# yancie-yjr/StreamYOLO

Measured on AMD Instinct MI355X. Metric: frame-pairs/sec (600x960) StreamYOLO-l fwd+bwd, higher is better.
Workload: dtype bf16; 1 GPU; StreamYOLO-l 600x960 training step: dual-frame forward + TAL loss + backward, 8 frame pairs/GPU/step, random-init synthetic weights (utils/synth.py); per_gpu_batch=8, global_batch=8, parallelism=dp1, hipgraph=False, launch_tape=True, optimizer_in_step=False, u8_input=False

## Files before the change

### streamyolo_amd/csrc/api_misc.hip

```cpp
#include "sy_device.h"
#include "../../include/streamyolo_hip.h"

extern "C" const char* sy_version(void) {
#ifdef SY_EMU
    return "streamyolo-hip 0.1 (SIMT-EMULATOR TEST BUILD - not a product binary)";
#else
    return "streamyolo-hip 0.1 (gfx950)";
#endif
}
extern "C" int sy_abi_version(void) { return SY_ABI_VERSION; }

namespace {

template <typename T> __device__ __forceinline__ void put(void* base, long long i, float v) {
    reinterpret_cast<typename T::elem*>(base)[i] = T::from_f32(v);
}
template <typename T> __device__ __forceinline__ long long frag_index(int row, int tap, int c, int taps, int kc) {
    constexpr int EPC = T::kEPC, BK = 4 * EPC;
    const int cslab = c / BK, within = c % BK;
    const int g = within / (2 * EPC), half = (within / EPC) & 1, e = within % EPC;
    const int ct = row >> 5, r = row & 31, nslab = kc / BK;
    return ((((((long long)ct * nslab + cslab) * taps + tap) * 2 + g) * 2 + half) * 32 + r) * EPC + e;
}

constexpr int kPackTile = 32, kPackTaps = 9;

template <typename T> __device__ void pack_tile(const sy_pack_entry& e, int tile, float (*lds)[kPackTile][kPackTile + 1]) {
    const int tiles_ci = (e.ci_n + kPackTile - 1) / kPackTile;
    const int co0 = (tile / tiles_ci) * kPackTile, ci0 = (tile % tiles_ci) * kPackTile;
    const int taps = e.taps;
    const int a_l = threadIdx.x >> 5, b_l = threadIdx.x & 31;
    for (int pass = 0; pass < kPackTile / 8; ++pass) {
        const int col = a_l + 8 * pass, co = co0 + col, ci = ci0 + b_l;
        const bool ok = co < e.co_n && ci < e.ci_n;
        const float* src = e.w + ((long long)co * e.ci_n + ci) * taps;
        const int row = e.r0 + co;
        for (int t = 0; t < taps; ++t) {
            const float v = ok ? src[t] : 0.0f;
            lds[t][col][b_l] = v;
            if (!ok) continue;
            if (e.packed != nullptr) put<T>(e.packed, ((long long)row * taps + t) * e.CI + ci, v);
            if (e.frag != nullptr) put<T>(e.frag, frag_index<T>(row, t, ci, taps, e.CI), v);
        }
    }
    __syncthreads();
    if (e.packed_t == nullptr && e.frag_t == nullptr) return;
    for (int pass = 0; pass < kPackTile / 8; ++pass) {
        const int cil = a_l + 8 * pass, ci = ci0 + cil, co = co0 + b_l;
        if (co >= e.co_n || ci >= e.ci_n) continue;
        const int row = e.r0 + co;
        for (int t = 0; t < taps; ++t) {
            const float v = lds[t][b_l][cil];
            if (e.packed_t != nullptr) put<T>(e.packed_t, ((long long)ci * taps + t) * e.R_t + row, v);
            if (e.frag_t != nullptr) put<T>(e.frag_t, frag_index<T>(ci, t, row, taps, e.R_t), v);
        }
    }
}

__global__ __launch_bounds__(256) void pack_weights_kernel(const sy_pack_entry* entries, int n_entries) {
    SY_TL_BEGIN(15);
    __shared__ float lds[kPackTaps][kPackTile][kPackTile + 1];
    int lo = 0, hi = n_entries - 1;
    while (lo < hi) {
        const int mid = (lo + hi + 1) >> 1;
        if (entries[mid].tile0 <= (int)blockIdx.x) lo = mid; else hi = mid - 1;
    }
    const sy_pack_entry e = entries[lo];
    const int tile = (int)blockIdx.x - e.tile0;
    const int tiles = ((e.co_n + kPackTile - 1) / kPackTile) * ((e.ci_n + kPackTile - 1) / kPackTile);
    if (tile >= tiles || e.taps > kPackTaps) return;
    switch (e.dtype) {
        case SY_DT_BF16: pack_tile<BF16>(e, tile, lds); break;
        case SY_DT_F16: pack_tile<F16>(e, tile, lds); break;
        default: pack_tile<F32>(e, tile, lds); break;
    }
    SY_TL_END();
}

}

extern "C" int sy_pack_weights(const sy_pack_entry* entries, int n_entries, int total_tiles, void* stream) {
    if (entries == nullptr || n_entries <= 0 || total_tiles <= 0) return SY_ERR_ARG;
    SY_LAUNCH(pack_weights_kernel, dim3(total_tiles), dim3(256), 0, stream, entries, n_entries);
    return SY_LAUNCH_OK() == 0 ? SY_OK : SY_ERR_LAUNCH;
}

namespace {

__global__ __launch_bounds__(256) void rows_add_kernel(float* dst, long long ldd, float* src, long long lds, int rows, int cols,
                                                      int zero_src) {
    const long long total = (long long)rows * cols;
    for (long long i = (long long)blockIdx.x * 256 + threadIdx.x; i < total; i += (long long)gridDim.x * 256) {
        const long long r = i / cols, c = i - r * cols;
        dst[r * ldd + c] += src[r * lds + c];
        if (zero_src) src[r * lds + c] = 0.0f;
    }
}

__global__ __launch_bounds__(256) void pred_colsum_kernel(const float* d_raw, int B, long long bs, int rows, int nch, float* partial,
                                                         int nch_pad) {
    SY_TL_BEGIN(15);
    __shared__ float red[16][17];
    const int c = threadIdx.x & 15, rl = threadIdx.x >> 4, col = blockIdx.y * 16 + c;
    const long long total = (long long)B * rows;
    float acc = 0.0f;
    if (col < nch)
        for (long long i = (long long)blockIdx.x * 16 + rl; i < total; i += (long long)gridDim.x * 16) {
            const long long b = i / rows, p = i - b * rows;
            acc += d_raw[b * bs + p * nch + col];
        }
    red[rl][c] = acc;
    __syncthreads();
    if (rl == 0) {
        float s = 0.0f;
#pragma unroll
        for (int k = 0; k < 16; ++k) s += red[k][c];
        partial[(long long)blockIdx.x * nch_pad + col] = s;
    }
    SY_TL_END();
}

__global__ __launch_bounds__(256) void pred_fold_kernel(const float* partial, int G, int nch_pad, int nc, float* scratch, int srows, int ld, int cin,
                                                       float* g_reg, float* g_obj, float* g_cls, float* gb_reg, float* gb_obj,
                                                       float* gb_cls) {
    SY_TL_BEGIN(15);
    const int t = threadIdx.x;
    for (int col = t; col < 5 + nc; col += 256) {
        float s = 0.0f;
        for (int g = 0; g < G; ++g) s += partial[(long long)g * nch_pad + col];
        if (col < 4) gb_reg[col] += s;
        else if (col == 4) gb_obj[0] += s;
        else gb_cls[col - 5] += s;
    }
    float* s0 = scratch;
    float* s1 = scratch + srows * (long long)ld;
    for (int i = t; i < 5 * cin; i += 256) {
        const int r = i / cin, k = i - r * cin;
        const float v = s0[r * ld + k];
        s0[r * ld + k] = 0.0f;
        if (r < 4) g_reg[r * cin + k] += v; else g_obj[k] += v;
    }
    for (int i = t; i < nc * cin; i += 256) {
        const int r = i / cin, k = i - r * cin;
        g_cls[i] += s1[r * ld + k];
        s1[r * ld + k] = 0.0f;
    }
    SY_TL_END();
}

}

extern "C" int sy_rows_add_f32(float* dst, int64_t ldd, float* src, int64_t lds, int rows, int cols, int zero_src, void* stream) {
    if (dst == nullptr || src == nullptr || rows <= 0 || cols <= 0 || ldd < cols || lds < cols) return SY_ERR_ARG;
    long long blocks = ((long long)rows * cols + 255) / 256;
    if (blocks > 1024) blocks = 1024;
    SY_LAUNCH(rows_add_kernel, dim3((unsigned)blocks), dim3(256), 0, stream, dst, (long long)ldd, src, (long long)lds, rows, cols, zero_src);
    return SY_LAUNCH_OK() == 0 ? SY_OK : SY_ERR_LAUNCH;
}

extern "C" int64_t sy_pred_grad_fold_workspace_floats(int num_classes) {
    return 64LL * (((5 + num_classes) + 15) / 16 * 16);
}

extern "C" int sy_pred_grad_fold(const float* d_raw, int B, int64_t batch_stride, int rows, int num_classes, float* scratch,
                                 int scratch_rows, int ld, int cin, float* g_reg, float* g_obj, float* g_cls, float* gb_reg, float* gb_obj, float* gb_cls,
                                 float* workspace, void* stream) {
    if (d_raw == nullptr || scratch == nullptr || workspace == nullptr || g_reg == nullptr || g_obj == nullptr || g_cls == nullptr ||
        gb_reg == nullptr || gb_obj == nullptr || gb_cls == nullptr || B <= 0 || rows <= 0 || num_classes <= 0 || cin <= 0 || ld < cin || scratch_rows < 5 || scratch_rows < num_classes)
        return SY_ERR_ARG;
    const int nch = 5 + num_classes, groups = (nch + 15) / 16, nch_pad = groups * 16, G = 64;
    SY_LAUNCH(pred_colsum_kernel, dim3(G, groups), dim3(256), 0, stream, d_raw, B, (long long)batch_stride, rows, nch, workspace, nch_pad);
    SY_LAUNCH(pred_fold_kernel, dim3(1), dim3(256), 0, stream, (const float*)workspace, G, nch_pad, num_classes, scratch, scratch_rows, ld, cin, g_reg,
              g_obj, g_cls, gb_reg, gb_obj, gb_cls);
    return SY_LAUNCH_OK() == 0 ? SY_OK : SY_ERR_LAUNCH;
}
SY_PROBE_READER(sy_probe_read_api_misc)
```

### streamyolo_amd/train_engine.py

```python
import ctypes as C
import os

import torch

from . import ops
from .data import FramePairsU8
from .engine import _Builder, MergedConv, base_convs, build_frame_net, build_fuse_net, build_head_net
from .model.plan_cache import compute_dtype_for
from .ops import View, EPI_LINEAR, CONV_DGRAD


_FUSED_FINALIZE = __import__("os").environ.get("STREAMYOLO_FUSED_FINALIZE", "auto")
BNR_FUSION = __import__("os").environ.get("STREAMYOLO_BNR_FUSION", "0") != "0"
BNR_TILES = (98, 100, 101, 109, 104, 107, 117, 118)
EXACT_STATS = __import__("os").environ.get("STREAMYOLO_EXACT_STATS", "1") != "0"
BN_BAPPLY_BLOCKS_SCHEDULED = 512


def _schedule_bn_caps():
    if os.environ.get("SY_BN_BAPPLY_BLOCKS"):
        return ops.bn_grid_caps()["bwd_reduce"]
    return ops.bn_grid_caps(bwd_apply=BN_BAPPLY_BLOCKS_SCHEDULED)["bwd_reduce"]


def exact_stat_rows(N, H, W):
    return N * H * ((W + 31) // 32)



class _GradSpace:

    def __init__(self):
        self.mirror = {}
        self.written = {}
        self.py = lambda fn: fn()

    def reset(self):
        self.written = {}

    def view(self, v):
        if v.root is not None:
            full, n0 = v.root
            gf = self.mirror.get(id(full))
            if gf is None:
                gf = torch.empty_like(full)
                self.mirror[id(full)] = gf
            return View(gf[n0:n0 + v.N], v.N, v.H, v.W, v.C, v.ld, v.c_off, v.bs_, root=(gf, n0))
        g = self.mirror.get(id(v.buf))
        if g is None:
            g = torch.empty_like(v.buf)
            self.mirror[id(v.buf)] = g
        return View(g, v.N, v.H, v.W, v.C, v.ld, v.c_off, v.bs_)

    def target(self, v):
        key = (id(v.root[0]), v.root[1]) if v.root is not None else id(v.buf)
        iv = self.written.setdefault(key, [])
        c0, c1 = v.c_off, v.c_off + v.C
        assert v.bs_ is None and c1 <= v.ld
        gaps, pos = [], c0
        for a, b in iv:
            if b <= pos or a >= c1:
                continue
            if a > pos:
                gaps.append((pos, a))
            pos = max(pos, b)
        if pos < c1:
            gaps.append((pos, c1))
        g = self.view(v)
        if len(gaps) == 1 and gaps[0] == (c0, c1):
            accumulate = False
        else:
            accumulate = True
            flat = g.buf.view(-1, v.ld)
            for a, b in gaps:
                ops.zero(flat[:, a:b])
        if gaps:
            merged = []
            for a, b in sorted(iv + [(c0, c1)]):
                if merged and a <= merged[-1][1]:
                    merged[-1] = (merged[-1][0], max(merged[-1][1], b))
                else:
                    merged.append((a, b))
            iv[:] = merged
        return g, accumulate


class _PairBuilder(_Builder):

    def __init__(self, dtype, device):
        super().__init__(dtype, device)
        self.fulls, self.replay, self.paired = [], None, True

    def buf(self, N, H, W, C):
        if not self.paired:
            return super().buf(N, H, W, C)
        if self.replay is None:
            full = torch.empty((2 * N, H, W, C), dtype=ops.TORCH_DTYPE[ops.dtype_code(self.dtype)], device=self.device)
            self.fulls.append(full)
            half = 0
        else:
            full = self.fulls[self.replay]
            self.replay += 1
            half = 1
            assert tuple(full.shape) == (2 * N, H, W, C)
        return View(full[half * N:(half + 1) * N], N, H, W, C, root=(full, half * N))


class StagedWeights:

    def __init__(self, plan_ops, dtype, device):
        from . import _lib
        self.dtype, self.device = dtype, device
        tdt = ops.TORCH_DTYPE[dtype]
        epc = 16 // torch.empty(0, dtype=tdt).element_size()
        bk = 4 * epc
        self.conv, self.preds, self.sources = {}, {}, []
        rows = []

        def z(n, dt=tdt):
            return torch.zeros(n, dtype=dt, device=device)

        def entry(w, packed, packed_t, frag, frag_t, co_n, ci_n, taps, r0, R, R_t, CI, dt=dtype):
            e = _lib.PackEntry()
            e.w = w.data_ptr()
            e.packed, e.packed_t = _ptr(packed), _ptr(packed_t)
            e.frag, e.frag_t = _ptr(frag), _ptr(frag_t)
            e.co_n, e.ci_n, e.taps, e.r0, e.R, e.R_t, e.CI, e.dtype = co_n, ci_n, taps, r0, R, R_t, CI, dt
            rows.append(e)
            self.sources.append(w)

        def _ptr(t):
            return None if t is None else t.data_ptr()

        self.bn = {}
        for op in plan_ops:
            if op.kind == "conv" and id(op.mod) not in self.conv:
                parts = base_convs(op.mod)
                w0 = parts[0].conv.weight
                ci, kh, kw = w0.shape[1:]
                co = sum(m.conv.weight.shape[0] for m in parts)
                taps, CI = kh * kw, (16 if ci == 12 else ci)
                packed, packed_t = z(co * taps * CI).view(co, taps * CI), z(CI * taps * co).view(CI, taps * co)
                frag = z(-(-co // 32) * 32 * taps * CI) if CI % bk == 0 else None
                frag_t = z(-(-CI // 32) * 32 * taps * co) if co % bk == 0 else None
                r0 = 0
                for m in parts:
                    w = m.conv.weight
                    assert w.dtype == torch.float32 and w.is_contiguous() and tuple(w.shape[1:]) == (ci, kh, kw)
                    entry(w, packed, packed_t, frag, frag_t, w.shape[0], ci, taps, r0, co, co, CI)
                    r0 += w.shape[0]
                self.conv[id(op.mod)] = (packed, packed_t, frag, frag_t)
                if len(parts) > 1:
                    gs, bs_ = z(co, torch.float32), z(co, torch.float32)
                    r0 = 0
                    for m in parts:
                        c = m.bn.weight.numel()
                        entry(m.bn.weight, gs, None, None, None, c, 1, 1, r0, co, co, 1, ops.DTYPE_NAME["fp32"])
                        entry(m.bn.bias, bs_, None, None, None, c, 1, 1, r0, co, co, 1, ops.DTYPE_NAME["fp32"])
                        r0 += c
                    self.bn[id(op.mod)] = (gs, bs_)
            elif op.kind == "pred":
                cin, nc = op.reg_mod.weight.shape[1], op.cls_mod.weight.shape[0]
                w_ro, w_ro_t = z(5 * cin).view(5, cin), z(cin * 8).view(cin, 8)
                w_c, w_c_t = z(nc * cin).view(nc, cin), z(cin * nc).view(cin, nc)
                b_ro = z(5, torch.float32)
                entry(op.reg_mod.weight, w_ro, w_ro_t, None, None, 4, cin, 1, 0, 5, 8, cin)
                entry(op.obj_mod.weight, w_ro, w_ro_t, None, None, 1, cin, 1, 4, 5, 8, cin)
                entry(op.cls_mod.weight, w_c, w_c_t, None, None, nc, cin, 1, 0, nc, nc, cin)
                entry(op.reg_mod.bias, b_ro, None, None, None, 4, 1, 1, 0, 5, 5, 1, ops.DTYPE_NAME["fp32"])
                entry(op.obj_mod.bias, b_ro, None, None, None, 1, 1, 1, 4, 5, 5, 1, ops.DTYPE_NAME["fp32"])
                self.preds[id(op)] = (w_ro, b_ro, w_c, op.cls_mod.bias, w_ro_t, w_c_t)
        arr, tiles = _lib.pack_table(rows)
        self.table = (torch.frombuffer(bytearray(bytes(arr)), dtype=torch.uint8).to(device), len(rows), tiles)
        self.n = len(rows)
        self.sig = tuple(t.data_ptr() for t in self.sources)

    def valid(self):
        return self.sig == tuple(t.data_ptr() for t in self.sources)

    def refresh(self):
        table, n, tiles = self.table
        ops.check(ops._lib.lib().sy_pack_weights(table.data_ptr(), n, tiles, ops.stream_of(table)), "sy_pack_weights")

    def conv_weight(self, mod, transpose=False):
        return self.conv[id(mod)][1 if transpose else 0]

    def conv_weight_frag(self, mod, transpose=False):
        return self.conv[id(mod)][3 if transpose else 2]

    def pred(self, op):
        w_ro, b_ro, w_c, b_c, w_ro_t, w_c_t = self.preds[id(op)]
        return w_ro, b_ro, w_c, b_c.detach(), w_ro_t, w_c_t


CSP_FORK = os.environ.get("STREAMYOLO_CSP_FORK", "1") != "0"
MERGE_SIBLINGS_TRAIN = os.environ.get("STREAMYOLO_MERGE_TRAIN", "1") != "0"
FWD_SPLIT_FRAMES = os.environ.get("STREAMYOLO_FWD_SPLIT_FRAMES", "1") != "0"
BWD_SPLIT_FRAMES = os.environ.get("STREAMYOLO_BWD_SPLIT_FRAMES", "auto")
HEAD_BWD_CHAINS = os.environ.get("STREAMYOLO_HEAD_BWD_CHAINS", "1") != "0"
HEAD_EARLY = os.environ.get("STREAMYOLO_HEAD_EARLY", "1") != "0"
CHAIN_SLOT_DONE = os.environ.get("STREAMYOLO_CHAIN_SLOT_DONE", "0") != "0"
SLOT_BATCH = max(1, int(os.environ.get("STREAMYOLO_SLOT_BATCH", "3")))
DUAL_WGRAD = os.environ.get("STREAMYOLO_DUAL_WGRAD", "1") != "0"
WGRAD_STREAMS = [1, 3, 4, 5][:max(1, min(4, int(os.environ.get("STREAMYOLO_WGRAD_STREAMS", "2")) if DUAL_WGRAD else 1))]


NINE_TAP_WGRAD_TILES = (52, 59, 60)


def scheduled_wgrad(wt, cin, env=None):
    env = os.environ if env is None else env
    tile, blocks = wt
    cap = int(env.get("STREAMYOLO_WGRAD_BLOCKS_CAP", "512"))
    if cap > 0 and blocks > cap:
        blocks = cap
    if tile in NINE_TAP_WGRAD_TILES:
        cap9 = int(env.get("STREAMYOLO_WGRAD9_BLOCKS", "128"))
        wide9 = int(env.get("STREAMYOLO_WGRAD9_WIDE", "60"))
        if wide9 and cin % 64 == 0:
            tile, cap9 = wide9, int(env.get("STREAMYOLO_WGRAD9_WIDE_BLOCKS", "96"))
        if cap9 > 0 and blocks > cap9:
            blocks = cap9
    return (tile, blocks)


def _csp_role(tag):
    head, _, leaf = tag.rpartition(".")
    if leaf not in ("conv2", "conv3") or ".m." in tag or head in ("", "spp"):
        return None
    return leaf


class TrainPlan:
    BWD_COPIES = int(os.environ.get("STREAMYOLO_BWD_COPIES", "2"))
    STAT_COPIES = int(os.environ.get("STREAMYOLO_STAT_COPIES", "0"))
    WGRAD_WS_BYTES = 256 << 20
    RING = int(os.environ.get("STREAMYOLO_RING", "0"))
    STREAMS = int(os.environ.get("STREAMYOLO_STREAMS", "2"))
    TAPE_ON_CPU = True

    def __init__(self, model, B, H, W, dtype, device, parts="full", feat_shapes=None, pool=None):
        self.model, self.B, self.H, self.W, self.device = model, B, H, W, device
        self.parts = parts
        self.pool = pool
        self.dtype = ops.dtype_code(dtype)
        self.tdtype = ops.TORCH_DTYPE[self.dtype]
        pafpn = model.backbone if parts == "full" else (model if parts == "backbone" else None)
        head = model.head if parts == "full" else (model if parts == "head" else None)
        self.head = head
        self.cache = None
        b = _PairBuilder(self.dtype, device)
        b.merge_siblings = MERGE_SIBLINGS_TRAIN
        if pafpn is not None:
            self.f0_cur, cur = build_frame_net(b, pafpn, B, H, W)
            self.n_frame_ops = len(b.ops)
            b.replay = 0
            self.f0_sup, sup = build_frame_net(b, pafpn, B, H, W)
            assert len(b.ops) == 2 * self.n_frame_ops and b.replay == len(b.fulls)
            b.paired = False
            fused = build_fuse_net(b, pafpn, cur, sup)
        else:
            self.n_frame_ops = 0
            b.paired = False
            fused = tuple(b.buf(B, h, w, c) for c, h, w in feat_shapes)
        self.fused = fused
        self.n_head_start = len(b.ops)
        self.preds, self.A = (build_head_net(b, head, fused) if head is not None else ([], 0))
        lvl = 0
        for op in b.ops[self.n_head_start:]:
            op.level = lvl
            lvl += 1 if op.kind == "pred" else 0
        self.hw = [(f.H, f.W) for f in fused]
        self.ops = b.ops
        self.nc = head.num_classes if head is not None else 0
        nch = 5 + self.nc
        self.raw = torch.empty((B, self.A, nch), dtype=torch.float32, device=device)
        self.dpad = torch.zeros((B, self.A, 16), dtype=self.tdtype, device=device)

        convs = [op for op in self.ops if op.kind == "conv"]
        tot_c = sum(op.y.C for op in convs)
        self.exact_stats = EXACT_STATS
        self.stat_copies = self.STAT_COPIES if self.STAT_COPIES > 0 else (32 if self.dtype == ops.DT_F32 else 4)
        self.fused_finalize = ((_FUSED_FINALIZE == "1") or (_FUSED_FINALIZE == "auto" and self.dtype != ops.DT_F32)) and not self.exact_stats
        reduce_cap = _schedule_bn_caps()

        def copies_of(op):
            if not self.exact_stats:
                return self.stat_copies, self.BWD_COPIES
            return max(self.stat_copies, exact_stat_rows(op.y.N, op.y.H, op.y.W)), max(self.BWD_COPIES, reduce_cap)
        for op in convs:
            op.stat_copies, op.bwd_copies = copies_of(op)
        self.stat_arena = torch.zeros(2 * sum(op.stat_copies * op.y.C for op in convs), dtype=torch.float32, device=device)
        self.bwd_arena = torch.zeros(2 * sum(op.bwd_copies * op.y.C for op in convs), dtype=torch.float32, device=device)
        self.aff_arena = torch.empty(4 * tot_c, dtype=torch.float32, device=device)
        sq0 = self.stat_arena.numel() // 2
        off = 0
        max_raw = 0
        nf = self.n_frame_ops
        for i in range(nf):
            a, b2 = self.ops[i], self.ops[nf + i]
            if a.kind == "conv":
                full = torch.empty((2 * a.y.N, a.y.H, a.y.W, a.y.C), dtype=self.tdtype, device=device)
                a.yraw = View(full[:a.y.N], a.y.N, a.y.H, a.y.W, a.y.C, root=(full, 0))
                b2.yraw = View(full[a.y.N:], a.y.N, a.y.H, a.y.W, a.y.C, root=(full, a.y.N))
        units = [(self.ops[i], self.ops[nf + i]) for i in range(nf) if self.ops[i].kind == "conv"]
        units += [(op,) for op in self.ops[2 * nf:] if op.kind == "conv"]
        s_off = b_off = 0
        for unit in units:
            C, S = unit[0].y.C, len(unit)
            SC, BC = unit[0].stat_copies, unit[0].bwd_copies
            u_sum = self.stat_arena[s_off:s_off + SC * S * C]
            u_sq = self.stat_arena[sq0 + s_off:sq0 + s_off + SC * S * C]
            u_bsum = self.bwd_arena[b_off:b_off + 2 * BC * S * C]
            s_off += SC * S * C
            b_off += 2 * BC * S * C
            u_aff = tuple(self.aff_arena[k * tot_c + off:k * tot_c + off + S * C] for k in range(4))
            for s_, op in enumerate(unit):
                op.stat = (u_sum[s_ * SC * C:(s_ + 1) * SC * C], u_sq[s_ * SC * C:(s_ + 1) * SC * C])
                op.bsum = u_bsum[s_ * 2 * BC * C:(s_ + 1) * 2 * BC * C]
                op.aff = tuple(t[s_ * C:(s_ + 1) * C] for t in u_aff)
                if op.yraw is None:
                    op.yraw = View.alloc(op.y.N, op.y.H, op.y.W, C, self.dtype, device)
                max_raw = max(max_raw, 2 * op.y.pixels * C)
            unit[0].unit = (u_sum, u_sq, u_bsum, u_aff)
            off += S * C
        self.max_raw = max_raw
        self._bind_scratch()
        self.ring_i = 0
        self.side = torch.cuda.Stream(device=device) if (device.type == "cuda" and self.STREAMS > 1) else None
        w_ = float(getattr(pafpn, "width", 1.0)) if pafpn is not None else 0.0
        self.bwd_split = (BWD_SPLIT_FRAMES == "1") or (BWD_SPLIT_FRAMES == "auto" and B * H * W * w_ * w_ >= 2.0e6)
        self.side2 = torch.cuda.Stream(device=device) if (self.side is not None and (self.bwd_split or HEAD_BWD_CHAINS)) else None
        self.side_w = {k: torch.cuda.Stream(device=device) for k in WGRAD_STREAMS[1:]} if self.side is not None else {}
        self.side3 = self.side_w.get(3)
        self._chain, self._wg_stream, self._wg_flip = 0, 1, 0
        self.tuned = False
        self.force_serial = False
        self._ev_pool = []
        for op in self.ops:
            if op.kind == "spp":
                op.argmax = torch.empty((op.v.N, op.v.H, op.v.W, 3, op.v.C // 4), dtype=torch.uint8, device=device)
        self.cache = StagedWeights(self.ops, self.dtype, device)
        self.loss_ws = None
        self._zeroed, self._zero_ev, self._packed_for = None, None, None
        self.run_table = None
        self.grads = _GradSpace()
        self.grads.py = self._py
        self.programs, self._rec, self._param_sig = {}, None, None
        self._side_region = False
        self.pending = 0

        group_of = {}
        for op in self.ops:
            if op.kind == "conv" and isinstance(op.mod, MergedConv):
                parts = base_convs(op.mod)
                block = [m.conv.weight for m in parts] + [m.bn.weight for m in parts] + [m.bn.bias for m in parts]
                for t in block:
                    group_of[id(t)] = block
        self.params, seen = [], set()
        for p in model.parameters():
            if not p.requires_grad or id(p) in seen:
                continue
            for t in group_of.get(id(p), (p,)):
                assert t.requires_grad and id(t) not in seen
                seen.add(id(t))
                self.params.append(t)
        n = sum(p.numel() for p in self.params)
        self.arena = torch.zeros(n, dtype=torch.float32, device=device)
        self.gview = {}
        o = 0
        for p in self.params:
            self.gview[id(p)] = self.arena[o:o + p.numel()].view(p.shape)
            o += p.numel()
        self._build_buckets()
        self.on_bucket = None
        self.bn_mods = [m.bn for op in convs for m in base_convs(op.mod)]
        self.stem_scratch = None
        self.pred_scratch = torch.zeros((2, max(8, self.nc), int(256 * head.width)), dtype=torch.float32, device=device) \
            if head is not None else None
        self.pred_ws = torch.empty(int(ops._lib.lib().sy_pred_grad_fold_workspace_floats(self.nc)), dtype=torch.float32,
                                   device=device) if head is not None else None

    def _bind_scratch(self):
        esz = torch.empty(0, dtype=self.tdtype).element_size()
        ring_bytes = -(-self.max_raw * esz // 256) * 256
        if self.pool is not None:
            self.wgrad_ws = self.pool.shared_scratch("wgrad_ws", self.WGRAD_WS_BYTES, self.device)
            slots = [self.pool.shared_scratch("dyraw_ring_%d" % i, ring_bytes, self.device) for i in range(max(self.RING, 0))]
            self._scratch_gen = self.pool.scratch_gen
        else:
            self.wgrad_ws = torch.empty(self.WGRAD_WS_BYTES, dtype=torch.uint8, device=self.device)
            slots = [torch.empty(ring_bytes, dtype=torch.uint8, device=self.device) for _ in range(max(self.RING, 0))]
            self._scratch_gen = 0
        self.dyraw_ring = [t[:self.max_raw * esz].view(self.tdtype) for t in slots]
        self.dyraw_own = []
        self.wgrad_ws_by = {WGRAD_STREAMS[0]: self.wgrad_ws}
        for k in WGRAD_STREAMS[1:]:
            self.wgrad_ws_by[k] = (self.pool.shared_scratch("wgrad_ws%d" % k, self.WGRAD_WS_BYTES, self.device)
                                   if self.pool is not None else torch.empty(self.WGRAD_WS_BYTES, dtype=torch.uint8, device=self.device))
        if self.pool is not None:
            self._scratch_gen = self.pool.scratch_gen

    def release(self):
        self.programs.clear()
        self.dyraw_own = []
        self.grads.py = None
        self.grads.mirror.clear()
        self.on_bucket = None

    def forward(self, x):
        if self.parts != "head":
            x = x.float().contiguous()
        if self.pool is not None and self._scratch_gen != self.pool.scratch_gen:
            self._bind_scratch()
            self.programs.clear()
        sig = tuple(p.data_ptr() for p in self.params)
        if sig != self._param_sig or not self.cache.valid():
            self._param_sig = sig
            self.programs.clear()
            if not self.cache.valid():
                self.cache = StagedWeights(self.ops, self.dtype, self.device)
        self.cache.refresh()
        ops.zero(self.stat_arena)
        if self.parts == "head":
            for v, t in zip(self.fused, x):
                assert tuple(t.shape) == (v.N, v.C, v.H, v.W)
                v.set_nchw(t.detach())
        elif isinstance(x, FramePairsU8):
            x.pack_focus(self.f0_cur, self.f0_sup)
        else:
            ops.focus_pack(x, 0, self.f0_cur)
            ops.focus_pack(x, 3, self.f0_sup)
        self._run("fwd", self._forward_ops)
        if self.run_table is None or not self.run_table.valid():
            mods = {}
            for op in self.ops:
                if op.kind == "conv":
                    c0, ctot, SC = 0, op.y.C, (32 if op.stat_copies > 64 else op.stat_copies)
                    for m in base_convs(op.mod):
                        mods.setdefault(id(m.bn), (m.bn, []))[1].append((op.stat[0][c0:], op.stat[1][c0:], op.y.pixels, SC, ctot))
                        c0 += m.bn.num_features
            self.run_table = ops.BnRunningTable(list(mods.values()), self.device, count_batches=True)
        self.run_table.run()
        return self.raw if self.head is not None else self.fused

    def _forward_ops(self):
        nf = self.n_frame_ops
        if FWD_SPLIT_FRAMES and nf:
            early = self._early_levels() if (HEAD_EARLY and self.head is not None and self.side2 is not None) else {}
            self._mark("fork")
            for i in range(nf):
                self._forward_op(self.ops[i])
                self._mark("side_nw")
                self._forward_op(self.ops[nf + i])
                self._mark("main", None)
                for lvl_ops in early.get(i, ()):
                    self._mark("dep", (0, 2))
                    self._mark("dep", (1, 2))
                    self._mark("cur", 2)
                    for op in lvl_ops:
                        self._forward_op(op)
                    self._mark("cur", 0)
            self._mark("join")
            if early:
                done = {id(op) for v in early.values() for lvl_ops in v for op in lvl_ops}
                for op in self.ops[2 * nf:]:
                    if id(op) not in done:
                        self._forward_op(op)
                self._mark("dep", (2, 0))
                return
        for i in range(nf if not (FWD_SPLIT_FRAMES and nf) else 0):
            a, b2 = self.ops[i], self.ops[nf + i]
            if a.kind == "conv":
                role = _csp_role(a.tag) if CSP_FORK else None
                if role == "conv2":
                    self._mark("side")
                    self._forward_pair(a)
                    self._mark("main", None)
                    continue
                if role == "conv3":
                    self._mark("join")
                self._forward_pair(a)
            else:
                self._forward_op(a)
                self._forward_op(b2)
        for op in self.ops[2 * nf:self.n_head_start]:
            self._forward_op(op)
        self._mark("fork")
        for op in self.ops[self.n_head_start:]:
            if op.level == 0:
                self._forward_op(op)
        self._mark("side_nw")
        self._side_region = True
        for op in self.ops[self.n_head_start:]:
            if op.level != 0:
                self._forward_op(op)
        self._side_region = False
        self._mark("main", None)
        self._mark("join")

    def _early_levels(self):
        nf = self.n_frame_ops
        fuse = self.ops[2 * nf:self.n_head_start]
        head_ops = self.ops[self.n_head_start:]
        nlev = len(self.preds)
        if len(fuse) != 2 * nlev:
            return {}
        out = {}
        for k in range(nlev):
            src = fuse[2 * k].x.buf.data_ptr()
            writers = [i for i in range(nf) if self.ops[i].kind == "conv" and self.ops[i].y.buf.data_ptr() == src]
            if not writers or max(writers) >= nf - 1:
                continue
            out.setdefault(max(writers), []).append([fuse[2 * k], fuse[2 * k + 1]] + [op for op in head_ops if op.level == k])
        return out

    def _bn_params(self, op):
        parts = base_convs(op.mod)
        bn = parts[0].bn
        mom = bn.momentum if bn.momentum is not None else 0.1
        if len(parts) == 1:
            return bn.weight, bn.bias, bn.eps, mom
        assert all(m.bn.eps == bn.eps and m.bn.momentum == bn.momentum for m in parts)
        g, b_ = self.cache.bn[id(op.mod)]
        return g, b_, bn.eps, mom

    def _bn_bwd(self, op, y, da, aff, gamma, bsum, dy, dgamma, dbeta, nseg=1, dres=None, acc=False, atomic=False):
        fused = getattr(op, "bnr_by", None) is not None
        if not fused:
            ops.bn_silu_bwd_reduce(y, da, *aff, bsum, nseg=nseg)
        ops.bn_silu_bwd_apply(y, da, *aff, gamma, bsum, dy, dgamma, dbeta, nseg=nseg, dres=dres, dres_accumulate=acc,
                              atomic_param_grads=atomic, raw_moment=fused)

    def _bnr_producer(self, op, dx, acc, t):
        pre = op.pre_op
        if (not BNR_FUSION or pre is None or acc or self.dtype == ops.DT_F32 or t not in BNR_TILES or op.k != 3 or op.stride != 1
                or pre.res is not None or pre.yraw is None or pre.yraw.ld != dx.ld or pre.yraw.bs != dx.bs or pre.y.C % 8 or dx.ld % 8
                or (dx.ptr() | pre.yraw.ptr()) % 16 or dx.bs % 8):
            return None
        return pre

    def _bn_grads(self, op):
        bn = base_convs(op.mod)[0].bn
        return self.gview[id(bn.weight)], self.gview[id(bn.bias)]

    def _forward_pair(self, a):
        gamma, beta, eps, mom = self._bn_params(a)
        x2, raw2, y2 = a.x.pair(), a.yraw.pair(), a.y.pair()
        u_sum, u_sq, _, (scale, shift, mean, invstd) = a.unit
        t = a._tiles.get("fwd_stats2")
        if t is None:
            t = ops.tuned_tile(ops.CONV_FWD, x2.dtype, x2.N, x2.H, x2.W, x2.C, y2.C, a.k, a.stride, self.device,
                               with_stats=True)
            a._tiles["fwd_stats2"] = t
        ops.conv2d(x2, self.cache.conv_weight(a.mod), raw2, a.k, a.stride, stats=(u_sum, u_sq), tile=t,
                   wfrag=self.cache.conv_weight_frag(a.mod) if t >= ops.TILE_WR else None, segments=2)
        if self.fused_finalize:
            ops.bn_finalize_apply(u_sum, u_sq, a.y.pixels, gamma, beta, eps, scale, shift, mean, invstd, raw2, y2,
                                  res=None if a.res is None else a.res.pair(), nseg=2)
        else:
            ops.bn_finalize(u_sum, u_sq, a.y.pixels, gamma, beta, eps, mom, None, None, scale, shift, mean, invstd,
                            nseg=2)
            ops.bn_silu_apply(raw2, scale, shift, y2, res=None if a.res is None else a.res.pair(), nseg=2)

    def _mark(self, kind, arg=None):
        if self._rec is not None:
            self._rec.mark(kind, arg)

    def _py(self, fn):
        fn()
        if self._rec is not None:
            self._rec.snippet(fn)

    def _run(self, name, body, key=None):
        from . import _lib
        if self.force_serial or not self.tuned or self.device.type != "cuda" and not self.TAPE_ON_CPU:
            self._rec = None
            body()
            return
        prog = self.programs.get(name)
        if prog is None or prog[0] != key:
            tape = _lib.NativeTape()
            with tape:
                self._rec = tape
                try:
                    body()
                finally:
                    self._rec = None
            self.programs[name] = (key, tape)
            return
        self._interpret(prog[1])

    def _interpret(self, tape):
        side, side2 = self.side, self.side2
        extra = [self.side_w.get(k) for k in (3, 4, 5)]
        if self.device.type == "cuda":
            main = torch.cuda.current_stream(self.device)
            main_h = C.c_void_p(main.cuda_stream)
            side_h = C.c_void_p(side.cuda_stream) if side is not None else None
            more = [C.c_void_p(st_.cuda_stream) if st_ is not None else None for st_ in [side2] + extra]
            while more and more[-1] is None:
                more.pop()
            if torch.cuda.is_current_stream_capturing():
                more = []
        else:
            main, main_h, side_h, more = None, C.c_void_p(0), None, []
        chains = [main, side, side2] + extra

        def snippet(fn, k):
            if k and chains[k] is not None:
                with torch.cuda.stream(chains[k]):
                    fn()
            else:
                fn()
        on_bucket = None
        if self.on_bucket is not None:
            on_bucket = lambda k: self.on_bucket(k, main, [s_ for s_ in [side, side2] + extra if s_ is not None])
        tape.replay(main_h, side_h, snippet, on_bucket, more=more)

    def _forward_op(self, op):
        nch = 5 + self.nc
        k = op.kind
        if k == "conv":
            gamma, beta, eps, mom = self._bn_params(op)
            w = self.cache.conv_weight(op.mod)
            t = op.tile("fwd_stats")
            scale, shift, mean, invstd = op.aff
            ops.conv2d(op.x, w, op.yraw, op.k, op.stride, stats=op.stat, tile=t,
                       wfrag=self.cache.conv_weight_frag(op.mod) if t >= ops.TILE_WR else None)
            if self.fused_finalize:
                ops.bn_finalize_apply(op.stat[0], op.stat[1], op.y.pixels, gamma, beta, eps, scale, shift, mean, invstd,
                                      op.yraw, op.y, res=op.res)
            else:
                ops.bn_finalize(op.stat[0], op.stat[1], op.y.pixels, gamma, beta, eps, mom,
                                None, None, scale, shift, mean, invstd)
                ops.bn_silu_apply(op.yraw, scale, shift, op.y, res=op.res)
        elif k == "resize":
            ops.resize_nearest(op.src, op.dst)
        elif k == "spp":
            ops.spp_pool(op.v, op.argmax)
        else:
            w_ro, b_ro, w_c, b_c = self.cache.pred(op)[:4]
            base = self.raw.data_ptr() + op.a0 * nch * 4
            ops.conv2d(op.reg_x, w_ro, None, 1, 1, None, b_ro, epilogue=EPI_LINEAR, y_f32=True, y_ptr=base,
                       y_ld=nch, y_bs=self.A * nch, cout=5)
            ops.conv2d(op.cls_x, w_c, None, 1, 1, None, b_c, epilogue=EPI_LINEAR, y_f32=True, y_ptr=base + 20,
                       y_ld=nch, y_bs=self.A * nch, cout=self.nc)

    def loss(self, labels, support, scaler=None):
        head = self.head
        if self.loss_ws is None or self.loss_ws.max_labels != labels.shape[1]:
            self.loss_ws = ops.TalLossWorkspace(self.B, self.A, 5 + self.nc, self.hw, head.strides, self.device,
                                                max_labels=labels.shape[1])
        pad = self.dpad if self.nc <= 8 else None
        self._zero_gradient_arenas()
        losses, d_raw, _ = ops.tal_loss(self.raw, labels, support, self.nc, head.gamma, head.ignore_thr,
                                        head.ignore_value, head.use_l1, self.loss_ws, d_pad=pad,
                                        scaler_state=None if scaler is None else scaler.state(self.device))
        self._packed_for = (d_raw, d_raw._version) if pad is not None else None
        out = {"total_loss": losses[0], "iou_loss": losses[1], "l1_loss": losses[2], "conf_loss": losses[3],
               "cls_loss": losses[4], "num_fg": losses[5]}
        return out, d_raw

    def backward(self, d_raw, d_fused=None):
        self._zero_gradient_arenas(wait=True)
        nc = self.nc
        pf = getattr(self, "_packed_for", None)
        if self.head is not None and not (pf is not None and pf[0] is d_raw and pf[1] == d_raw._version):
            self.dpad[..., 0:5] = d_raw[..., 0:5]
            self.dpad[..., 8:8 + nc] = d_raw[..., 5:]
        self._packed_for = None
        self._seed = d_fused
        self._run("bwd", lambda: self._backward_ops(d_raw), key=None if d_raw is None else d_raw.data_ptr())
        if not self.tuned:
            self.tuned = True
            ops.save_tuned()
        return self.arena

    def _zero_gradient_arenas(self, wait=False):
        st = self.side_w.get(3) or self.side2 or self.side
        if wait:
            if self._zeroed is None:
                ops.zero(self.arena)
                ops.zero(self.bwd_arena)
            elif self._zeroed is not True:
                torch.cuda.current_stream(self.device).wait_event(self._zeroed)
            self._zeroed = None
            return
        if self._zeroed is not None:
            return
        if st is None or self.device.type != "cuda" or torch.cuda.is_current_stream_capturing():
            ops.zero(self.arena)
            ops.zero(self.bwd_arena)
            self._zeroed = True
            return
        st.wait_stream(torch.cuda.current_stream(self.device))
        with torch.cuda.stream(st):
            ops.zero(self.arena)
            ops.zero(self.bwd_arena)
            if self._zero_ev is None:
                self._zero_ev = torch.cuda.Event()
            self._zero_ev.record()
        self._zeroed = self._zero_ev

    def fused_grads(self):
        return tuple(self.grads.view(f).nchw() for f in self.fused)

    BUCKET_BYTES = 32 << 20
    FIRST_BUCKET_BYTES = 4 << 20

    def _backward_sequence(self):
        nf = self.n_frame_ops
        return list(reversed(self.ops[2 * nf:])) + [self.ops[i] for i in reversed(range(nf))]

    def _build_buckets(self):
        last = {}
        for pos, op in enumerate(self._backward_sequence()):
            if op.kind == "conv":
                prm = tuple(t for m in base_convs(op.mod) for t in (m.conv.weight, m.bn.weight, m.bn.bias))
            elif op.kind == "pred":
                prm = tuple(t for m in (op.reg_mod, op.obj_mod, op.cls_mod) for t in (m.weight, m.bias))
            else:
                prm = ()
            for t in prm:
                last[id(t)] = pos
        self.buckets, lo, o, ready = [], 0, 0, -1
        for p in self.params:
            o += p.numel()
            ready = max(ready, last.get(id(p), -1))
            if (o - lo) * 4 >= (self.BUCKET_BYTES if self.buckets else min(self.FIRST_BUCKET_BYTES, self.BUCKET_BYTES)):
                self.buckets.append((lo, o, ready))
                lo, ready = o, -1
        if o > lo:
            self.buckets.append((lo, o, ready))
        self.bucket_at = {}
        for k, (_, _, r) in enumerate(self.buckets):
            self.bucket_at.setdefault(r, []).append(k)

    def _bucket_marks(self, pos):
        for k in self.bucket_at.get(pos, ()):
            self._mark("bucket", k)

    def _backward_ops(self, d_raw):
        G = self.grads
        G.reset()
        for op in self.ops:
            if op.kind == "conv":
                op.bnr_by = None
        self.ring_i = 0
        self._split_j = 0
        nf = self.n_frame_ops
        if self.head is None:
            for i, f in enumerate(self.fused):
                gv, acc = G.target(f)
                assert not acc
                self._py(lambda gv=gv, i=i: gv.set_nchw(self._seed[i]))
        self._bucket_marks(-1)
        split = self.bwd_split and nf > 0
        self._chain, self._wg_flip = 0, 0
        head_chain = HEAD_BWD_CHAINS and self.head is not None and self.side2 is not None
        n_head = len(self.ops) - self.n_head_start
        if head_chain:
            self._mark("dep", (0, 2))
        for pos, a in enumerate(self._backward_sequence()):
            if head_chain and pos == n_head:
                self._chain = 0
                self._mark("cur", 0)
                self._mark("dep", (2, 0))
            if split and pos == len(self.ops) - 2 * nf:
                self._mark("dep", (0, 2))
            if pos < len(self.ops) - 2 * nf:
                if head_chain and pos < n_head:
                    k = 2 if a.level != 0 else 0
                    if k != self._chain:
                        self._chain = k
                        self._mark("cur", k)
                if a.kind == "pred":
                    self._pred_backward(a, d_raw)
                else:
                    self._conv_backward(a)
            else:
                b2 = self.ops[nf + (len(self.ops) - 2 * nf) + nf - 1 - pos]
                if a.kind == "conv":
                    if split:
                        self._conv_pair_backward_split(a, b2)
                    else:
                        self._conv_pair_backward(a, b2)
                else:
                    for op in (b2, a):
                        if split:
                            self._mark("cur", 2 if op is b2 else 0)
                        if op.kind == "resize":
                            dsrc, acc = G.target(op.src)
                            ops.resize_nearest_bwd(G.view(op.dst), dsrc, acc)
                        elif op.kind == "spp":
                            ops.spp_pool_bwd(G.view(op.v), op.argmax)
            self._bucket_marks(pos)
        if split:
            self._mark("cur", 0)
            self._mark("dep", (2, 0))
        for k in WGRAD_STREAMS:
            if k != 1:
                self._mark("dep", (k, 0))
        self._mark("join")

    def _scratch(self, numel):
        if self.RING <= 0:
            self._slot = None
            return self._own_buffer(numel)
        self.ring_i = (self.ring_i + 1) % self.RING
        self._slot = self.ring_i
        self._mark("acquire_cur", self._slot)
        return self.dyraw_ring[self._slot][:numel]

    def _own_buffer(self, numel):
        i = self.ring_i
        self.ring_i += 1
        if i == len(self.dyraw_own):
            self.dyraw_own.append(torch.empty(numel, dtype=self.tdtype, device=self.device))
        assert self.dyraw_own[i].numel() >= numel
        return self.dyraw_own[i][:numel]

    def _wgrad_stream(self, fixed=None):
        if fixed is not None:
            return fixed
        self._wg_flip = (self._wg_flip + 1) % len(WGRAD_STREAMS)
        return WGRAD_STREAMS[self._wg_flip]

    def _on_side(self, fn, slot=None, chains=None, stream=None):
        chains = (self._chain,) if chains is None else chains
        w = self._wgrad_stream(stream)
        for k in chains:
            self._mark("dep", (k, w))
        self._mark("cur", w)
        self._wg_stream = w
        fn()
        self._wg_stream = 1
        if slot is not None:
            self._mark("slot_done", slot)
        self._mark("cur", self._chain)

    def _ws(self):
        return self.wgrad_ws_by[self._wg_stream]

    def _pred_backward(self, op, d_raw):
        G = self.grads
        hwk = op.reg_x.H * op.reg_x.W
        B, A, nc = self.B, self.A, self.nc
        w_ro_t, w_c_t = self.cache.pred(op)[4:6]
        d_ro = View(self.dpad, B, op.reg_x.H, op.reg_x.W, 8, 16, op.a0 * 16, bs=A * 16)
        d_c = View(self.dpad, B, op.reg_x.H, op.reg_x.W, nc, 16, op.a0 * 16 + 8, bs=A * 16)
        g_r, acc_r = G.target(op.reg_x)
        ops.conv2d(d_ro, w_ro_t, g_r, 1, 1, mode=CONV_DGRAD, accumulate=acc_r)
        g_c, acc_c = G.target(op.cls_x)
        ops.conv2d(d_c, w_c_t, g_c, 1, 1, mode=CONV_DGRAD, accumulate=acc_c)
        cin = op.reg_x.C

        sc = self.pred_scratch
        g_reg, g_obj, g_cls = (self.gview[id(m.weight)] for m in (op.reg_mod, op.obj_mod, op.cls_mod))
        gb_r, gb_o, gb_c = (self.gview[id(m.bias)] for m in (op.reg_mod, op.obj_mod, op.cls_mod))

        def wg():
            ops.conv2d_wgrad(op.reg_x, d_ro, sc[0], 1, 1, workspace=self._ws())
            ops.conv2d_wgrad(op.cls_x, d_c, sc[1], 1, 1, workspace=self._ws())
            ops.pred_grad_fold(d_raw, op.a0, hwk, nc, sc, cin, g_reg, g_obj, g_cls, gb_r, gb_o, gb_c, self.pred_ws)
        self._on_side(wg, stream=1)

    def _bn_backward(self, op, dyraw):
        G = self.grads
        gamma = self._bn_params(op)[0]
        dgamma, dbeta = self._bn_grads(op)
        dY = G.view(op.y)
        dres, acc = (None, False) if op.res is None else G.target(op.res)
        scale, shift, mean, invstd = op.aff
        self._bn_bwd(op, op.yraw, dY, (scale, shift, mean, invstd), gamma, op.bsum, dyraw, dgamma, dbeta, dres=dres, acc=acc)

    def _wgrad(self, op, x, dyraw):
        w = base_convs(op.mod)[0].conv.weight
        key = "wgrad%d" % x.N
        wt = op._tiles.get(key)
        if wt is None:
            wt = ops.tuned_wgrad(x.dtype, x.N, x.H, x.W, x.C, dyraw.H, dyraw.W, dyraw.C, op.k, op.stride,
                                 self.device, self.wgrad_ws)
            wt = scheduled_wgrad(wt, x.C)
            op._tiles[key] = wt
        if w.shape[1] == x.C:
            ops.conv2d_wgrad(x, dyraw, self.gview[id(w)], op.k, op.stride, oihw=True, workspace=self._ws(),
                             tile=wt[0], target_blocks=wt[1])
        else:
            if self.stem_scratch is None:
                self.stem_scratch = torch.zeros((w.shape[0], x.C, op.k, op.k), dtype=torch.float32, device=self.device)
            sc, gw = self.stem_scratch, self.gview[id(w)]
            ops.conv2d_wgrad(x, dyraw, sc, op.k, op.stride, oihw=True, workspace=self._ws(),
                             tile=wt[0], target_blocks=wt[1])
            kk = op.k * op.k
            ops.rows_add_f32(gw, sc, w.shape[0], w.shape[1] * kk, w.shape[1] * kk, x.C * kk, zero_src=True)

    def _conv_pair_backward(self, a, b2):
        G = self.grads
        N, H, W, C = a.y.N, a.y.H, a.y.W, a.y.C
        full = self._scratch(2 * N * H * W * C).view(2 * N, H, W, C)
        slot = self._slot
        dy2 = View(full, 2 * N, H, W, C)
        gamma = self._bn_params(a)[0]
        dgamma, dbeta = self._bn_grads(a)
        dYa, dYb = G.view(a.y), G.view(b2.y)
        assert dYa.root[0] is dYb.root[0]
        dY2 = dYa.pair()
        dres2, acca = None, False
        if a.res is not None:
            dra, acca = G.target(a.res)
            drb, accb = G.target(b2.res)
            assert acca == accb and dra.root[0] is drb.root[0]
            dres2 = dra.pair()
        _, _, u_bsum, (scale, shift, mean, invstd) = a.unit
        raw2 = a.yraw.pair()
        self._bn_bwd(a, raw2, dY2, (scale, shift, mean, invstd), gamma, u_bsum, dy2, dgamma, dbeta, nseg=2, dres=dres2, acc=acca)
        self._on_side(lambda: self._wgrad(a, a.x.pair(), dy2), slot)
        if a.need_dx:
            dxa, acca = G.target(a.x)
            dxb, accb = G.target(b2.x)
            assert acca == accb and dxa.root[0] is dxb.root[0]
            t = a._tiles.get("dgrad2")
            if t is None:
                t = ops.tuned_tile(CONV_DGRAD, dy2.dtype, 2 * N, H, W, C, a.x.C, a.k, a.stride, self.device)
                a._tiles["dgrad2"] = t
            ops.conv2d(dy2, self.cache.conv_weight(a.mod, transpose=True), dxa.pair(), a.k, a.stride,
                       mode=CONV_DGRAD, accumulate=acca, tile=t,
                       wfrag=self.cache.conv_weight_frag(a.mod, transpose=True) if t >= ops.TILE_WR else None)
            if slot is not None:
                self._mark("slot_done", slot)

    def _conv_pair_backward_split(self, a, b2):
        G = self.grads
        N, H, W, C = a.y.N, a.y.H, a.y.W, a.y.C
        if self.RING <= 0:
            slot, full = None, self._own_buffer(2 * N * H * W * C).view(2 * N, H, W, C)
        else:
            self.ring_i = (self.ring_i + 1) % self.RING
            slot = self.ring_i
            full = self.dyraw_ring[slot][:2 * N * H * W * C].view(2 * N, H, W, C)
        dy2 = View(full, 2 * N, H, W, C)
        dys = (View(full[:N], N, H, W, C), View(full[N:], N, H, W, C))
        gamma = self._bn_params(a)[0]
        dgamma, dbeta = self._bn_grads(a)
        j, K = self._split_j, max(1, min(SLOT_BATCH, self.RING - 2))
        self._split_j += 1
        batched = K > 1 and j >= self.RING
        for k, (op, dyr) in enumerate(zip((a, b2), dys)):
            self._mark("cur", 2 * k)
            if slot is None:
                pass
            elif not batched:
                self._mark("acquire_cur", slot)
            elif (j - self.RING) % K == 0:
                for m in range(min(K, len(WGRAD_STREAMS))):
                    self._mark("acquire_cur", (slot + K - 1 - m) % self.RING)
            dres, acc = (None, False) if op.res is None else G.target(op.res)
            scale, shift, mean, invstd = op.aff
            self._bn_bwd(op, op.yraw, G.view(op.y), (scale, shift, mean, invstd), gamma, op.bsum, dyr, dgamma, dbeta,
                         dres=dres, acc=acc, atomic=True)
        self._chain = 0
        self._on_side(lambda: self._wgrad(a, a.x.pair(), dy2), slot, chains=(0, 2))
        if a.need_dx:
            t = a.tile("dgrad")
            for k, (op, dyr) in enumerate(zip((a, b2), dys)):
                self._mark("cur", 2 * k)
                dx, acc = G.target(op.x)
                pre = self._bnr_producer(op, dx, acc, t)
                if pre is not None:
                    pre.bnr_by = op
                ops.conv2d(dyr, self.cache.conv_weight(a.mod, transpose=True), dx, a.k, a.stride, mode=CONV_DGRAD,
                           accumulate=acc, tile=t,
                           wfrag=self.cache.conv_weight_frag(a.mod, transpose=True) if t >= ops.TILE_WR else None,
                           bn_reduce=None if pre is None else (pre.yraw, pre.aff[0], pre.aff[1], pre.bsum))
                if CHAIN_SLOT_DONE and slot is not None:
                    self._mark("slot_done", slot)
        self._mark("cur", 0)

    def _conv_backward(self, op):
        G = self.grads
        C = op.y.C
        dyraw = View(self._scratch(op.y.pixels * C).view(op.y.N, op.y.H, op.y.W, C), op.y.N, op.y.H, op.y.W, C)
        slot = self._slot
        self._bn_backward(op, dyraw)
        self._on_side(lambda: self._wgrad(op, op.x, dyraw), slot)
        if op.need_dx:
            dx, acc = G.target(op.x)
            t = op.tile("dgrad")
            ops.conv2d(dyraw, self.cache.conv_weight(op.mod, transpose=True), dx, op.k, op.stride,
                       mode=CONV_DGRAD, accumulate=acc, tile=t,
                       wfrag=self.cache.conv_weight_frag(op.mod, transpose=True) if t >= ops.TILE_WR else None)
            if slot is not None:
                self._mark("slot_done", slot)

    def profile(self, x, targets, iters=2, detail=False):
        evs = []
        real = {n: getattr(ops, n) for n in ("conv2d", "conv2d_wgrad", "bn_finalize", "bn_silu_apply", "bn_finalize_apply",
                                             "bn_silu_bwd_reduce", "bn_silu_bwd_apply", "resize_nearest",
                                             "resize_nearest_bwd", "spp_pool", "spp_pool_bwd", "view_copy", "focus_pack")}

        def wrap(name, fn):
            def inner(*a, **k):
                kind = name
                if name == "conv2d":
# ... 342 lines not shown
```

Baseline: 353.0 frame-pairs/s.

## Vectorize weight packing kernel and clear BN stat arena ahead on side stream

```diff
diff --git a/streamyolo_amd/csrc/api_misc.hip b/streamyolo_amd/csrc/api_misc.hip
--- a/streamyolo_amd/csrc/api_misc.hip
+++ b/streamyolo_amd/csrc/api_misc.hip
@@ -1,5 +1,6 @@
 #include "sy_device.h"
 #include "../../include/streamyolo_hip.h"
+#include <type_traits>
 
 extern "C" const char* sy_version(void) {
 #ifdef SY_EMU
@@ -12,54 +13,154 @@
 
 namespace {
 
-template <typename T> __device__ __forceinline__ void put(void* base, long long i, float v) {
-    reinterpret_cast<typename T::elem*>(base)[i] = T::from_f32(v);
-}
-template <typename T> __device__ __forceinline__ long long frag_index(int row, int tap, int c, int taps, int kc) {
-    constexpr int EPC = T::kEPC, BK = 4 * EPC;
-    const int cslab = c / BK, within = c % BK;
-    const int g = within / (2 * EPC), half = (within / EPC) & 1, e = within % EPC;
-    const int ct = row >> 5, r = row & 31, nslab = kc / BK;
-    return ((((((long long)ct * nslab + cslab) * taps + tap) * 2 + g) * 2 + half) * 32 + r) * EPC + e;
-}
-
 constexpr int kPackTile = 32, kPackTaps = 9;
-
-template <typename T> __device__ void pack_tile(const sy_pack_entry& e, int tile, float (*lds)[kPackTile][kPackTile + 1]) {
+constexpr int kPackPitch = kPackTile + 2;
+constexpr int kPackTapStride = kPackTile * kPackPitch + 8;
+constexpr int kPackLds = kPackTaps * kPackTapStride;
+
+#ifdef SY_EMU
+#define SY_PACK_GLOBAL
+#else
+#define SY_PACK_GLOBAL __attribute__((address_space(1)))
+#endif
+typedef unsigned pack_u4 __attribute__((ext_vector_type(4)));
+typedef float pack_f4 __attribute__((ext_vector_type(4)));
+
+__device__ __forceinline__ bool pack_aligned16(const void* p) { return (reinterpret_cast<uintptr_t>(p) & 15u) == 0; }
+__device__ __forceinline__ int pack_min(int a, int b) { return a < b ? a : b; }
+__device__ __forceinline__ int pack_max(int a, int b) { return a > b ? a : b; }
+__device__ __forceinline__ int pack_lds(int t, int col, int c) { return t * kPackTapStride + col * kPackPitch + c; }
+
+template <typename T, int TAPS, int TSTEP>
+__device__ __forceinline__ void pack_emit(typename T::elem* dst, long long dstep, const float* src, int sstride, int t0, int taps, bool vec,
+                                          int lo, int hi) {
+    constexpr int EPC = T::kEPC, NT = ((TAPS ? TAPS : kPackTaps) + TSTEP - 1) / TSTEP;
+    if (!vec) {
+#pragma nounroll
+        for (int t = t0; t < taps; t += TSTEP, dst += dstep, src += TSTEP * kPackTapStride)
+#pragma nounroll
+            for (int k = lo; k < hi; ++k) dst[k] = T::from_f32(src[k * sstride]);
+        return;
+    }
+#pragma unroll
+    for (int n = 0; n < NT; ++n) {
+        if (t0 + n * TSTEP >= taps) continue;
+        const float* s = src + n * TSTEP * kPackTapStride;
+        float v[EPC];
+#pragma unroll
+        for (int k = 0; k < EPC; ++k) v[k] = s[k * sstride];
+        pack_u4 o;
+        if constexpr (sizeof(typename T::elem) == 2) {
+            o = pack_u4{T::pack2(v[0], v[1]), T::pack2(v[2], v[3]), T::pack2(v[EPC - 4], v[EPC - 3]), T::pack2(v[EPC - 2], v[EPC - 1])};
+        } else {
+            o = pack_u4{__builtin_bit_cast(unsigned, v[0]), __builtin_bit_cast(unsigned, v[1]), __builtin_bit_cast(unsigned, v[2]),
+                        __builtin_bit_cast(unsigned, v[3])};
+        }
+        *(SY_PACK_GLOBAL pack_u4*)(dst + n * dstep) = o;
+    }
+}
+
+template <typename T, int TAPS> __device__ void pack_tile(const sy_pack_entry& e, int tile, float* lds) {
+    typedef typename T::elem elem;
+    constexpr int EPC = T::kEPC, BK = 4 * EPC, PPT = kPackTile / EPC;
+    constexpr int PAIRS = kPackTile * PPT, TG = 256 / PAIRS;
     const int tiles_ci = (e.ci_n + kPackTile - 1) / kPackTile;
     const int co0 = (tile / tiles_ci) * kPackTile, ci0 = (tile % tiles_ci) * kPackTile;
-    const int taps = e.taps;
-    const int a_l = threadIdx.x >> 5, b_l = threadIdx.x & 31;
-    for (int pass = 0; pass < kPackTile / 8; ++pass) {
-        const int col = a_l + 8 * pass, co = co0 + col, ci = ci0 + b_l;
-        const bool ok = co < e.co_n && ci < e.ci_n;
-        const float* src = e.w + ((long long)co * e.ci_n + ci) * taps;
-        const int row = e.r0 + co;
-        for (int t = 0; t < taps; ++t) {
-            const float v = ok ? src[t] : 0.0f;
-            lds[t][col][b_l] = v;
-            if (!ok) continue;
-            if (e.packed != nullptr) put<T>(e.packed, ((long long)row * taps + t) * e.CI + ci, v);
-            if (e.frag != nullptr) put<T>(e.frag, frag_index<T>(row, t, ci, taps, e.CI), v);
+    const int taps = TAPS ? TAPS : e.taps, tid = threadIdx.x;
+    const int nco = pack_min(kPackTile, e.co_n - co0), nci = pack_min(kPackTile, e.ci_n - ci0);
+    {
+        const int len = nci * taps;
+        const long long off0 = ((long long)co0 * e.ci_n + ci0) * taps, pitch = (long long)e.ci_n * taps;
+        if (((off0 | pitch | (long long)len) & 3) == 0 && pack_aligned16(e.w)) {
+            constexpr int KMAX = TAPS ? TAPS : kPackTaps;
+            const int vpr = len >> 2, total = nco * vpr;
+            const SY_PACK_GLOBAL float* w = (const SY_PACK_GLOBAL float*)e.w + off0;
+            auto load = [&](auto vpr_c) __attribute__((always_inline)) {
+                pack_f4 v[KMAX];
+                int col[KMAX], j[KMAX];
+#pragma unroll
+                for (int k = 0; k < KMAX; ++k) {
+                    const int i = tid + 256 * k;
+                    col[k] = i / (int)vpr_c;
+                    j[k] = (i - col[k] * (int)vpr_c) * 4;
+                    if (i < total) v[k] = *(const SY_PACK_GLOBAL pack_f4*)(w + col[k] * pitch + j[k]);
+                }
+#pragma unroll
+                for (int k = 0; k < KMAX; ++k) {
+                    if (tid + 256 * k >= total) continue;
+                    int c = j[k] / taps, t = j[k] - c * taps;
+#pragma unroll
+                    for (int q = 0; q < 4; ++q) {
+                        lds[pack_lds(t, col[k], c)] = v[k][q];
+                        if (++t == taps) { t = 0; ++c; }
+                    }
+                }
+            };
+            if (TAPS > 0 && nci == kPackTile) load(std::integral_constant<int, 8 * (TAPS ? TAPS : 1)>());
+            else load(vpr);
+        } else {
+            const int total = nco * len;
+            for (int i = tid; i < total; i += 256) {
+                const int col = i / len, j = i - col * len;
+                const int c = j / taps, t = j - c * taps;
+                lds[pack_lds(t, col, c)] = e.w[off0 + col * pitch + j];
+            }
         }
     }
     __syncthreads();
+    const int th = tid / PAIRS, pr = tid % PAIRS;
+    if (e.packed != nullptr) {
+        const int p = pr % PPT, col = pr / PPT, cl = p * EPC, n = pack_min(EPC, nci - cl);
+        if (col < nco && n > 0)
+            pack_emit<T, TAPS, TG>((elem*)e.packed + ((long long)(e.r0 + co0 + col) * taps + th) * e.CI + ci0 + cl, (long long)TG * e.CI,
+                                   lds + pack_lds(th, col, cl), 1, th, taps, n == EPC && e.CI % EPC == 0 && pack_aligned16(e.packed), 0, n);
+    }
+    if (e.frag != nullptr) {
+        const int col = pr % kPackTile, p = pr / kPackTile, cl = p * EPC, n = pack_min(EPC, nci - cl);
+        if (col < nco && n > 0) {
+            const int row = e.r0 + co0 + col, ci = ci0 + cl, nslab = e.CI / BK;
+            const long long i = (((((long long)(row >> 5) * nslab + ci / BK) * taps + th) * 4 + (ci % BK) / EPC) * 32 + (row & 31)) * EPC;
+            pack_emit<T, TAPS, TG>((elem*)e.frag + i, (long long)TG * 128 * EPC, lds + pack_lds(th, col, cl), 1, th, taps,
+                                   n == EPC && pack_aligned16(e.frag), 0, n);
+        }
+    }
     if (e.packed_t == nullptr && e.frag_t == nullptr) return;
-    for (int pass = 0; pass < kPackTile / 8; ++pass) {
-        const int cil = a_l + 8 * pass, ci = ci0 + cil, co = co0 + b_l;
-        if (co >= e.co_n || ci >= e.ci_n) continue;
-        const int row = e.r0 + co;
-        for (int t = 0; t < taps; ++t) {
-            const float v = lds[t][b_l][cil];
-            if (e.packed_t != nullptr) put<T>(e.packed_t, ((long long)ci * taps + t) * e.R_t + row, v);
-            if (e.frag_t != nullptr) put<T>(e.frag_t, frag_index<T>(ci, t, row, taps, e.R_t), v);
-        }
-    }
+    const int row_lo = e.r0 + co0, row_hi = row_lo + nco;
+    const int pc0 = row_lo / EPC, npc = (row_hi + EPC - 1) / EPC - pc0;
+    const bool vec_pt = e.R_t % EPC == 0 && pack_aligned16(e.packed_t), vec_ft = pack_aligned16(e.frag_t);
+    const int nslab_t = e.R_t / BK;
+    auto emit_t = [&](auto tstep_c, int q, int cil, int t0, bool to_packed) __attribute__((always_inline)) {
+        constexpr int TSTEP = decltype(tstep_c)::value;
+        if (q >= npc || cil >= nci) return;
+        const int prow = (pc0 + q) * EPC, lo = pack_max(0, row_lo - prow), hi = pack_min(EPC, row_hi - prow);
+        const bool full = lo == 0 && hi == EPC;
+        const float* src = lds + pack_lds(t0, 0, cil) + (prow - row_lo) * kPackPitch;
+        const int ci = ci0 + cil;
+        if (to_packed) {
+            pack_emit<T, TAPS, TSTEP>((elem*)e.packed_t + ((long long)ci * taps + t0) * e.R_t + prow, (long long)TSTEP * e.R_t, src, kPackPitch,
+                                      t0, taps, full && vec_pt, lo, hi);
+        } else {
+            const long long i = (((((long long)(ci >> 5) * nslab_t + prow / BK) * taps + t0) * 4 + (prow % BK) / EPC) * 32 + (ci & 31)) * EPC;
+            pack_emit<T, TAPS, TSTEP>((elem*)e.frag_t + i, (long long)TSTEP * 128 * EPC, src, kPackPitch, t0, taps, full && vec_ft, lo, hi);
+        }
+    };
+    if (e.packed_t != nullptr) emit_t(std::integral_constant<int, TG>(), pr % PPT, pr / PPT, th, true);
+    if (e.frag_t != nullptr) emit_t(std::integral_constant<int, TG>(), pr / kPackTile, pr % kPackTile, th, false);
+    if (npc > PPT) {
+        if (e.packed_t != nullptr) emit_t(std::integral_constant<int, 8>(), PPT, tid & 31, tid >> 5, true);
+        if (e.frag_t != nullptr) emit_t(std::integral_constant<int, 8>(), PPT, tid & 31, tid >> 5, false);
+    }
+}
+
+template <typename T> __device__ __forceinline__ void pack_tile_taps(const sy_pack_entry& e, int tile, float* lds) {
+    if (e.taps == 9) pack_tile<T, 9>(e, tile, lds);
+    else if (e.taps == 1) pack_tile<T, 1>(e, tile, lds);
+    else pack_tile<T, 0>(e, tile, lds);
 }
 
 __global__ __launch_bounds__(256) void pack_weights_kernel(const sy_pack_entry* entries, int n_entries) {
     SY_TL_BEGIN(15);
-    __shared__ float lds[kPackTaps][kPackTile][kPackTile + 1];
+    __shared__ __attribute__((aligned(16))) float lds[kPackLds];
     int lo = 0, hi = n_entries - 1;
     while (lo < hi) {
         const int mid = (lo + hi + 1) >> 1;
@@ -70,9 +171,9 @@
     const int tiles = ((e.co_n + kPackTile - 1) / kPackTile) * ((e.ci_n + kPackTile - 1) / kPackTile);
     if (tile >= tiles || e.taps > kPackTaps) return;
     switch (e.dtype) {
-        case SY_DT_BF16: pack_tile<BF16>(e, tile, lds); break;
-        case SY_DT_F16: pack_tile<F16>(e, tile, lds); break;
-        default: pack_tile<F32>(e, tile, lds); break;
+        case SY_DT_BF16: pack_tile_taps<BF16>(e, tile, lds); break;
+        case SY_DT_F16: pack_tile_taps<F16>(e, tile, lds); break;
+        default: pack_tile_taps<F32>(e, tile, lds); break;
     }
     SY_TL_END();
 }
diff --git a/streamyolo_amd/train_engine.py b/streamyolo_amd/train_engine.py
--- a/streamyolo_amd/train_engine.py
+++ b/streamyolo_amd/train_engine.py
@@ -203,6 +203,7 @@
 SLOT_BATCH = max(1, int(os.environ.get("STREAMYOLO_SLOT_BATCH", "3")))
 DUAL_WGRAD = os.environ.get("STREAMYOLO_DUAL_WGRAD", "1") != "0"
 WGRAD_STREAMS = [1, 3, 4, 5][:max(1, min(4, int(os.environ.get("STREAMYOLO_WGRAD_STREAMS", "2")) if DUAL_WGRAD else 1))]
+STATS_CLEAR_AHEAD = os.environ.get("STREAMYOLO_STATS_CLEAR_AHEAD", "1") != "0"
 
 
 NINE_TAP_WGRAD_TILES = (52, 59, 60)
@@ -343,6 +344,7 @@
         self.cache = StagedWeights(self.ops, self.dtype, device)
         self.loss_ws = None
         self._zeroed, self._zero_ev, self._packed_for = None, None, None
+        self._stat_clean, self._stat_ev = None, None
         self.run_table = None
         self.grads = _GradSpace()
         self.grads.py = self._py
@@ -421,7 +423,11 @@
             if not self.cache.valid():
                 self.cache = StagedWeights(self.ops, self.dtype, self.device)
         self.cache.refresh()
-        ops.zero(self.stat_arena)
+        ev, self._stat_clean = self._stat_clean, None
+        if ev is not None and STATS_CLEAR_AHEAD and not torch.cuda.is_current_stream_capturing():
+            torch.cuda.current_stream(self.device).wait_event(ev)
+        else:
+            ops.zero(self.stat_arena)
         if self.parts == "head":
             for v, t in zip(self.fused, x):
                 assert tuple(t.shape) == (v.N, v.C, v.H, v.W)
@@ -701,6 +707,12 @@
             if self._zero_ev is None:
                 self._zero_ev = torch.cuda.Event()
             self._zero_ev.record()
+            if STATS_CLEAR_AHEAD:
+                ops.zero(self.stat_arena)
+                if self._stat_ev is None:
+                    self._stat_ev = torch.cuda.Event()
+                self._stat_ev.record()
+                self._stat_clean = self._stat_ev
         self._zeroed = self._zero_ev
 
     def fused_grads(self):
```

After: 354.8 frame-pairs/s (median of 6 runs). Within noise of the previous version (+0.5%).
